# rust-cv/cv

Measured on NVIDIA H100. Metric: vSLAM frames/s (AKAZE+match+RANSAC, 1080p ~5k kp) at 1/2/4/8 H100, higher is better.
Workload: dtype f32+f64

## Files before the change

cv_b200/csrc/akaze.cu:

```cuda
#include <math.h>
#include <stdarg.h>
#include <stdio.h>
#include <stdlib.h>
#include <string.h>
#include <algorithm>
#include <vector>
#include "akaze_kernels.cuh"
#include "common.cuh"

using namespace akz;

namespace {

struct EvoHost {
    int w = 0, h = 0;
    uint32_t octave = 0, sublevel = 0;
    double esigma = 0, etime = 0;
    uint32_t sigma = 0;
    float quat = 0;
    float norm = 0, middle = 0;
    std::vector<double> tau;
    size_t off = 0;
    bool new_octave = false;
};
// ... 65 lines not shown
    int ks = radius * 2 + 1;
    if (ks > MAXK) return -1;
    t->ks = ks;
    memset(t->k, 0, sizeof(t->k));
    gaussian_kernel_host(r, ks, t->k);
    return 0;
}

}

struct AkazeWorkspace {
    cvb_akaze_cfg cfg{};
    uint32_t w = 0, h = 0, batch = 0;
    std::vector<EvoHost> evo;
    EvoTable table{};
    size_t plane_floats = 0;
    size_t p0 = 0;
    unsigned capc = 0, capk = 0;
    Taps g0{}, g1{};
    float *img = nullptr;
    float *Lt = nullptr, *Lsm = nullptr, *Lx = nullptr, *Ly = nullptr, *Lflow = nullptr, *Ldet = nullptr;
    float *tmpA = nullptr, *tmpB = nullptr, *tmpC = nullptr;
    bool fuse_blur_scharr = true;
    bool fuse_det = true;
    double *g2 = nullptr;
    unsigned long long *gmax = nullptr;
    unsigned *hist = nullptr, *npoints = nullptr;
    double *kc = nullptr;
    float *inv_k = nullptr;
    int *evo_octave = nullptr;
    unsigned *rowcount = nullptr, *rowoff = nullptr, *ncand = nullptr;
    Cand *cand = nullptr;
    cvb_keypoint *cache = nullptr, *refined = nullptr, *sorted = nullptr;
    unsigned *ncache = nullptr, *nsorted = nullptr, *nvalid = nullptr, *rank = nullptr;
    unsigned char *keep = nullptr, *valid = nullptr, *ok = nullptr, *desc_tmp = nullptr;
    unsigned *overflow = nullptr;
    CUtensorMap *tmaps = nullptr;
    bool use_tma = false;
    int tma_mask = 3;
    SupScratch sup{};
    bool suppress_seq = false;
    bool suppress_par_only = false;
    unsigned *sup_fallback = nullptr;
    unsigned char *tile_evo = nullptr;
    MaskLayout mask_layout{};
    unsigned *extrema_mask = nullptr;
    bool deriv_v3 = true;
    OrientTables *ot = nullptr;
    DescTables *dt = nullptr;
    cvb_keypoint *kp_out = nullptr;
    unsigned char *desc_out = nullptr;
    unsigned *n_out = nullptr;
    unsigned cap_out = 0;
    std::vector<void *> allocs;
    bool has_run = false;
    cudaStream_t aux = nullptr;
    cudaEvent_t ev_fork[8] = {}, ev_join = nullptr;
    struct GraphEntry { const void *img; void *kp, *desc, *n; unsigned B, cap; cudaGraphExec_t exec; };
    std::vector<GraphEntry> graphs;
    uint64_t launches_per_graph = 0;
    bool use_graph = true;
    bool use_aux = true;
};

void akaze_workspace_free(AkazeWorkspace *ws) {
    if (!ws) return;
    for (auto &g : ws->graphs) cudaGraphExecDestroy(g.exec);
// ... 208 lines not shown
    if (ws && same_cfg(ws->cfg, *cfg) && ws->w == w && ws->h == h && ws->batch >= batch && ws->cap_out >= cap_out) return 0;
    if (ws) { cvb_wait(ctx, ctx->stream); akaze_workspace_free(ws); ctx->akaze = nullptr; }
    if (cfg->descriptor_channels < 1 || cfg->descriptor_channels > 3) return cvb_set_error(ctx, CVB_EINVAL, "descriptor_channels must be 1..3");
    if (cfg->contrast_factor_num_bins < 1 || cfg->contrast_factor_num_bins > 8192) return cvb_set_error(ctx, CVB_EUNSUPPORTED, "contrast_factor_num_bins must be 1..8192");
    if (cfg->num_sublevels < 1) return cvb_set_error(ctx, CVB_EINVAL, "num_sublevels must be >= 1");
    if (!(cfg->base_scale_offset > 0.0)) return cvb_set_error(ctx, CVB_EINVAL, "sigma must be > 0.0");
    ws = new AkazeWorkspace();
    ws->cfg = *cfg; ws->w = w; ws->h = h; ws->batch = batch; ws->cap_out = cap_out;
    int rc = build_workspace(ctx, ws, cfg, batch, w, h, cap_out);
    if (rc) { cvb_wait(ctx, ctx->stream); akaze_workspace_free(ws); return rc; }
    ctx->akaze = ws;
    return 0;
}

int build_workspace(cvb_ctx *ctx, AkazeWorkspace *ws, const cvb_akaze_cfg *cfg, uint32_t batch, uint32_t w, uint32_t h, unsigned cap_out) {
    int rc = plan_evolutions(ctx, ws);
    if (rc) return rc;
    if (make_gauss_taps((float)cfg->base_scale_offset, &ws->g0)) return cvb_set_error(ctx, CVB_EUNSUPPORTED, "base_scale_offset too large");
    make_gauss_taps(1.0f, &ws->g1);
    ws->p0 = (size_t)w * h;
    ws->capc = (unsigned)std::min<size_t>(std::max<size_t>(ws->p0 / 8, 4096), 1u << 20);
    ws->capk = (unsigned)std::min<size_t>(std::max<size_t>(ws->p0 / 32, 4096), 1u << 17);
    const size_t B = batch, PF = ws->plane_floats, R = (size_t)std::max(ws->table.total_rows, 1);
#define DA(p, n) do { rc = dalloc(ctx, ws, &ws->p, (n)); if (rc) return rc; } while (0)
    DA(img, B * ws->p0);
    DA(Lt, B * PF); DA(Lsm, B * PF); DA(Lx, B * PF); DA(Ly, B * PF); DA(Lflow, B * PF); DA(Ldet, B * PF);
    DA(tmpA, B * ws->p0); DA(tmpB, B * ws->p0); DA(tmpC, B * ws->p0);
    DA(g2, B * ws->p0);
    DA(gmax, B); DA(hist, B * cfg->contrast_factor_num_bins); DA(npoints, B); DA(kc, B); DA(inv_k, B * MAX_EVO);
    DA(evo_octave, MAX_EVO);
    DA(rowcount, B * R); DA(rowoff, B * R); DA(ncand, B);
    DA(cand, B * ws->capc);
    DA(cache, B * ws->capk); DA(refined, B * ws->capk); DA(sorted, B * ws->capk);
    DA(ncache, B); DA(nsorted, B); DA(nvalid, B); DA(rank, B * ws->capk);
    DA(keep, B * ws->capk); DA(valid, B * ws->capk); DA(ok, B * ws->capk); DA(desc_tmp, B * ws->capk * 64);
    DA(overflow, 1);
    {
        unsigned nbmax = 1;
        for (size_t i = 0; i < ws->evo.size(); i++) {
            float ratio = (float)(1u << ws->evo[i].octave), off = 0.5f * (ratio - 1.0f), size = ws->table.e[i].size;
            float cell = fmaxf(16.0f, ceilf(2.0f * size + 2.0f * off + 2.0f));
            unsigned nbx = (unsigned)((float)w / cell) + 3, nby = (unsigned)((float)h / cell) + 3;
            nbmax = std::max(nbmax, nbx * nby);
        }
        ws->sup.nbmax = nbmax;
        DA(sup.state, B * ws->capc); DA(sup.alive, B * ws->capc); DA(sup.rdy, B * ws->capc);
        DA(sup.key, B * ws->capc); DA(sup.rank, B * ws->capc); DA(sup.next, B * ws->capc);
        DA(sup.binA, B * nbmax); DA(sup.binB, B * nbmax);
        const char *env = getenv("CVB_SUPPRESS_SEQ");
        ws->suppress_seq = env && env[0] == '1';
        env = getenv("CVB_SUPPRESS_GLOBAL");
        ws->suppress_par_only = env && env[0] == '1';
        DA(sup_fallback, B);
        env = getenv("CVB_NO_GRAPH");
        ws->use_graph = !(env && env[0] == '1');
        env = getenv("CVB_NO_AUX_STREAM");
        ws->use_aux = !(env && env[0] == '1');
        env = getenv("CVB_NO_FUSE_BLUR");
        ws->fuse_blur_scharr = !(env && env[0] == '1');
        env = getenv("CVB_NO_FUSE_DET");
        ws->fuse_det = !(env && env[0] == '1');
        cudaStreamCreateWithFlags(&ws->aux, cudaStreamNonBlocking);
        for (auto &e : ws->ev_fork) cudaEventCreateWithFlags(&e, cudaEventDisableTiming);
        cudaEventCreateWithFlags(&ws->ev_join, cudaEventDisableTiming);
        cudaFuncSetAttribute(k_suppress_smem, cudaFuncAttributeMaxDynamicSharedMemorySize, (int)SUP_SMEM);
    }
    DA(ot, 1); DA(dt, 1);
    DA(tmaps, 3 * MAX_EVO);
    DA(kp_out, B * (size_t)cap_out); DA(desc_out, B * (size_t)cap_out * 64); DA(n_out, B);
#undef DA
    {
        const char *env = getenv("CVB_TMA");
        ws->use_tma = env ? env[0] == '1' : (CVB_TMA_DEFAULT != 0);
        if (const char *m = getenv("CVB_TMA_MASK")) ws->tma_mask = atoi(m);
        std::vector<CUtensorMap> hm(3 * MAX_EVO);
        memset(hm.data(), 0, sizeof(CUtensorMap) * hm.size());
        for (size_t i = 0; i < ws->evo.size() && ws->use_tma; i++) {
            const EvoHost &e = ws->evo[i];
            const int S = std::min<int>((int)e.sigma, 5);
            if ((int)e.sigma > 5) { ws->use_tma = false; break; }
            const float *src1 = (i == 0 ? ws->Lt : ws->Lsm) + e.off;
            const bool ok = make_tmap(&hm[i], src1, e.w, e.h, batch, PF, pitch3(S), SH3 + 2 * S)
                         && make_tmap(&hm[MAX_EVO + i], ws->Lx + e.off, e.w, e.h, batch, PF, pitch3(S), SH3 + 2 * S)
                         && make_tmap(&hm[2 * MAX_EVO + i], ws->Ly + e.off, e.w, e.h, batch, PF, pitch3(S), SH3 + 2 * S);
            if (!ok) ws->use_tma = false;
        }
        CVB_CUDA(ctx, cudaMemcpyAsync(ws->tmaps, hm.data(), sizeof(CUtensorMap) * hm.size(), cudaMemcpyHostToDevice, ctx->stream));
        CVB_CUDA(ctx, cvb_wait(ctx, ctx->stream));
    }
    {
        std::vector<unsigned char> te((size_t)std::max(ws->table.total_tiles, 1), 0);
        ws->deriv_v3 = true;
        for (size_t i = 0; i < ws->evo.size(); i++) {
            const int t0 = ws->table.e[i].tilebase, t1 = i + 1 < ws->evo.size() ? ws->table.e[i + 1].tilebase : ws->table.total_tiles;
            for (int t = t0; t < t1; t++) te[(size_t)t] = (unsigned char)i;
            if (ws->evo[i].sigma > 5) ws->deriv_v3 = false;
        }
        rc = dalloc(ctx, ws, &ws->tile_evo, te.size());
// ... 223 lines not shown
            cur = dst; cur_bs = dst_bs;
        }
    }
    if ((rc = issue_detector_response(octave_first, E))) return rc;
    if (forked) {
        CVB_CUDA(ctx, cudaEventRecord(ws->ev_join, ws->aux));
        CVB_CUDA(ctx, cudaStreamWaitEvent(st, ws->ev_join, 0));
    }
    {
        if (!fused_det) { CVB_PROF(ctx, "k_extrema_mask", 4.0 * ws->plane_floats * B);
        k_extrema_mask<<<dim3((unsigned)ws->table.total_tiles, 1, B), NT, 0, st>>>(ws->Ldet, PF, ws->table, ws->tile_evo, ws->mask_layout, thr,
                                                                                    ws->extrema_mask, ws->rowcount);
        CVB_LAUNCH_CHECK(ctx); }
        { CVB_PROF(ctx, "k_scan_rows", 0);
        k_scan_rows<<<B, 1024, 0, st>>>(ws->rowcount, ws->rowoff, ws->ncand, R);
        CVB_LAUNCH_CHECK(ctx); }
        { CVB_PROF(ctx, "k_extrema_emit", 0);
        k_extrema_emit<<<dim3(cdiv((unsigned)R * 32u, NT), 1, B), NT, 0, st>>>(ws->Ldet, PF, ws->table, ws->mask_layout, ws->extrema_mask, ws->rowcount,
                                                                                 ws->rowoff, ws->cand, ws->capc, ws->overflow);
        CVB_LAUNCH_CHECK(ctx); }
    }
    { CVB_PROF(ctx, "k_suppress", 0);
    if (ws->suppress_seq)
        k_suppress_seq<<<B, 1024, 0, st>>>(ws->cand, ws->ncand, ws->capc, ws->table, ws->cache, ws->ncache, ws->capk, ws->overflow);
    else {
        k_suppress_smem<<<B, 1024, SUP_SMEM, st>>>(ws->cand, ws->ncand, ws->rowoff, ws->capc, ws->table, ws->sup, ws->cache,
                                                   ws->ncache, ws->capk, ws->overflow, ws->sup_fallback);
        CVB_LAUNCH_CHECK(ctx);
        k_suppress_par<<<B, 1024, 0, st>>>(ws->cand, ws->ncand, ws->rowoff, ws->capc, ws->table, ws->sup, ws->cache, ws->ncache,
                                           ws->capk, ws->overflow, ws->suppress_par_only ? nullptr : ws->sup_fallback);
    }
    CVB_LAUNCH_CHECK(ctx); }
    const unsigned kp_blocks = (unsigned)ctx->num_sms * 2;
    const unsigned ichunks = std::min<unsigned>(cdiv(ws->capk, NT), 64u);
    CVB_CUDA(ctx, cudaMemsetAsync(ws->keep, 1, (size_t)B * ws->capk, st));
    { CVB_PROF(ctx, "k_filter_upper", 0);
    k_filter_upper<<<dim3(ichunks, 16, B), NT, 0, st>>>(ws->cache, ws->ncache, ws->capk, ws->keep);
    CVB_LAUNCH_CHECK(ctx); }
    { CVB_PROF(ctx, "k_refine_orient", 0);
    k_refine_orient<<<dim3(kp_blocks, B), NT, 0, st>>>(ws->cache, ws->ncache, ws->capk, ws->keep, ws->table, ws->Ldet, ws->Lx, ws->Ly, PF,
                                                       ws->ot, ws->refined, ws->valid);
    CVB_LAUNCH_CHECK(ctx); }
    CVB_CUDA(ctx, cudaMemsetAsync(ws->rank, 0, sizeof(unsigned) * (size_t)B * ws->capk, st));
    CVB_CUDA(ctx, cudaMemsetAsync(ws->nvalid, 0, sizeof(unsigned) * B, st));
    { CVB_PROF(ctx, "k_rank_sort", 0);
    k_rank_count<<<dim3(ichunks, 16, B), NT, 0, st>>>(ws->refined, ws->valid, ws->ncache, ws->capk, ws->rank);
    CVB_LAUNCH_CHECK(ctx);
    k_rank_scatter<<<dim3(ichunks, B), NT, 0, st>>>(ws->refined, ws->valid, ws->ncache, ws->capk, ws->rank,
                                                    (long long)ws->cfg.maximum_features, ws->sorted, ws->nvalid);
    CVB_LAUNCH_CHECK(ctx);
    k_clamp_count<<<cdiv(B, 32), 32, 0, st>>>(ws->nvalid, (long long)ws->cfg.maximum_features, ws->nsorted, (int)B);
    CVB_LAUNCH_CHECK(ctx); }
    { CVB_PROF(ctx, "k_descriptors", 0);
    k_descriptors<<<dim3((unsigned)ctx->num_sms * 8, B), DESC_WARPS * 32, 0, st>>>(ws->sorted, ws->nsorted, ws->capk, ws->table, ws->Lt, ws->Lx,
                                                     ws->Ly, PF, ws->dt, (int)ws->cfg.descriptor_channels,
                                                     (int)ws->cfg.descriptor_pattern_size, ws->desc_tmp, ws->ok);
    CVB_LAUNCH_CHECK(ctx); }
    { CVB_PROF(ctx, "k_compact_final", 0);
    k_compact_final<<<B, 1024, 0, st>>>(ws->sorted, ws->desc_tmp, ws->ok, ws->nsorted, ws->capk, kp_out, desc_out, cap_out, n_out,
                                        ws->overflow);
    CVB_LAUNCH_CHECK(ctx); }
    ws->has_run = true;
    return 0;
}

int run_extract(cvb_ctx *ctx, const float *images, unsigned B, cvb_keypoint *kp_out, unsigned char *desc_out,
                unsigned cap_out, unsigned *n_out) {
    AkazeWorkspace *ws = ctx->akaze;
    if (!ws->use_graph || ctx->prof || ws->evo.empty()) return run_extract_eager(ctx, images, B, kp_out, desc_out, cap_out, n_out);
    for (auto &g : ws->graphs)
        if (g.img == images && g.kp == kp_out && g.desc == desc_out && g.n == n_out && g.B == B && g.cap == cap_out) {
            CVB_CUDA(ctx, cudaGraphLaunch(g.exec, ctx->stream));
            ctx->launches += ws->launches_per_graph;
            ws->has_run = true;
            return 0;
        }
    const uint64_t l0 = ctx->launches;
    cudaGraph_t graph = nullptr;
    CVB_CUDA(ctx, cudaStreamBeginCapture(ctx->stream, cudaStreamCaptureModeThreadLocal));
    int rc = run_extract_eager(ctx, images, B, kp_out, desc_out, cap_out, n_out);
    cudaError_t ce = cudaStreamEndCapture(ctx->stream, &graph);
    if (rc) { if (graph) cudaGraphDestroy(graph); return rc; }
    if (ce != cudaSuccess || !graph) {
        cudaGetLastError();
// ... 59 lines not shown
    CVB_CUDA(ctx, cudaMemcpyAsync(hs, ws->overflow, sizeof(unsigned), cudaMemcpyDeviceToHost, ctx->stream));
    CVB_CUDA(ctx, cudaMemsetAsync(ws->overflow, 0, sizeof(unsigned), ctx->stream));
    CVB_CUDA(ctx, cvb_wait(ctx, ctx->stream));
    *flag_out = hs[0];
    return 0;
}

int cvb_akaze_extract_batch(cvb_ctx *ctx, const cvb_akaze_cfg *cfg, const float *images, uint32_t batch, uint32_t w, uint32_t h,
                            cvb_keypoint *kp_out, uint8_t *desc_out, uint32_t cap, uint32_t *n_out) {
    return akaze_extract_batch_host(ctx, cfg, images, false, batch, w, h, kp_out, desc_out, cap, n_out);
}

}

int akaze_extract_batch_host(cvb_ctx *ctx, const cvb_akaze_cfg *cfg, const float *images, bool images_on_device, uint32_t batch, uint32_t w,
                             uint32_t h, cvb_keypoint *kp_out, uint8_t *desc_out, uint32_t cap, uint32_t *n_out) {
    int rc = check_args(ctx, cfg, images, batch, w, h);
    if (rc) return rc;
    if (!n_out || (cap && (!kp_out || !desc_out))) return cvb_set_error(ctx, CVB_EINVAL, "null output");
    CVB_CUDA(ctx, cudaSetDevice(ctx->device));
    rc = ensure_workspace(ctx, cfg, batch, w, h, std::max<uint32_t>(cap, 1));
    if (rc) return rc;
    AkazeWorkspace *ws = ctx->akaze;
    cudaStream_t st = ctx->stream;
    if (!images_on_device) CVB_CUDA(ctx, cudaMemcpyAsync(ws->img, images, sizeof(float) * ws->p0 * batch, cudaMemcpyHostToDevice, st));
    const unsigned cap_dev = ws->cap_out;
    rc = run_extract(ctx, images_on_device ? images : ws->img, batch, ws->kp_out, ws->desc_out, cap_dev, ws->n_out);
    if (rc) return rc;
    unsigned *hs = (unsigned *)cvb_pinned(ctx, sizeof(unsigned) * ((size_t)batch + 1));
    if (!hs) return cvb_set_error(ctx, CVB_ENOMEM, "page-locked scratch");
    CVB_CUDA(ctx, cudaMemcpyAsync(hs, ws->n_out, sizeof(unsigned) * batch, cudaMemcpyDeviceToHost, st));
    CVB_CUDA(ctx, cudaMemcpyAsync(hs + batch, ws->overflow, sizeof(unsigned), cudaMemcpyDeviceToHost, st));
    CVB_CUDA(ctx, cvb_wait(ctx, st));
    const unsigned ovf = hs[batch];
    for (uint32_t b = 0; b < batch; b++) n_out[b] = hs[b];
    if (ovf) {
        cudaMemsetAsync(ws->overflow, 0, sizeof(unsigned), st);
        if (ovf == 3) return cvb_set_error(ctx, CVB_ECAP, "output capacity %u too small", cap);
        return cvb_set_error(ctx, CVB_ECAP, "internal keypoint capacity exceeded (stage %u)", ovf);
    }
    for (uint32_t b = 0; b < batch; b++) {
        unsigned n = std::min<unsigned>(n_out[b], cap);
        if (!n) continue;
        CVB_CUDA(ctx, cudaMemcpyAsync(kp_out + (size_t)b * cap, ws->kp_out + (size_t)b * cap_dev, sizeof(cvb_keypoint) * n,
                                      cudaMemcpyDeviceToHost, st));
        CVB_CUDA(ctx, cudaMemcpyAsync(desc_out + (size_t)b * cap * 64, ws->desc_out + (size_t)b * cap_dev * 64, (size_t)n * 64,
                                      cudaMemcpyDeviceToHost, st));
    }
    CVB_CUDA(ctx, cvb_wait(ctx, st));
    return 0;
}

extern "C" {

int cvb_akaze_extract(cvb_ctx *ctx, const cvb_akaze_cfg *cfg, const float *image, uint32_t w, uint32_t h, cvb_keypoint *kp_out,
                      uint8_t *desc_out, uint32_t cap, uint32_t *n_out) {
    return cvb_akaze_extract_batch(ctx, cfg, image, 1, w, h, kp_out, desc_out, cap, n_out);
}

int cvb_akaze_debug_num_evolutions(cvb_ctx *ctx, uint32_t *n_out) {
    if (!ctx || !n_out) return CVB_EINVAL;
    if (!ctx->akaze || !ctx->akaze->has_run) return cvb_set_error(ctx, CVB_EINVAL, "no extract call yet");
    *n_out = (uint32_t)ctx->akaze->evo.size();
    return 0;
}

int cvb_akaze_debug_evolution(cvb_ctx *ctx, uint32_t i, uint32_t *w, uint32_t *h, uint32_t *octave, uint32_t *sigma_size,
                              uint32_t *n_fed_steps) {
// ... 45 lines not shown
        if (n) CVB_CUDA(ctx, cudaMemcpy(c.data(), ws->cand + (size_t)frame * ws->capc, sizeof(Cand) * n, cudaMemcpyDeviceToHost));
        for (unsigned i = 0; i < n; i++) {
            cvb_keypoint k{};
            const EvoHost &e = ws->evo[(size_t)c[i].e];
            k.x = (float)c[i].x; k.y = (float)c[i].y; k.response = fabsf(c[i].v);
            k.size = (float)(e.esigma * ws->cfg.derivative_factor); k.angle = 0.f; k.octave = e.octave; k.class_id = (uint32_t)c[i].e;
            res.push_back(k);
        }
    } else if (stage == 1 || stage == 2) {
        unsigned n = 0;
        CVB_CUDA(ctx, cudaMemcpy(&n, ws->ncache + frame, sizeof(unsigned), cudaMemcpyDeviceToHost));
        std::vector<cvb_keypoint> k(n);
        std::vector<unsigned char> f(n);
        const cvb_keypoint *src = stage == 1 ? ws->cache : ws->refined;
        const unsigned char *flg = stage == 1 ? ws->keep : ws->valid;
        if (n) {
            CVB_CUDA(ctx, cudaMemcpy(k.data(), src + (size_t)frame * ws->capk, sizeof(cvb_keypoint) * n, cudaMemcpyDeviceToHost));
            CVB_CUDA(ctx, cudaMemcpy(f.data(), flg + (size_t)frame * ws->capk, n, cudaMemcpyDeviceToHost));
        }
        for (unsigned i = 0; i < n; i++)
            if (f[i]) res.push_back(k[i]);
    } else if (stage == 3) {
        unsigned n = 0;
        CVB_CUDA(ctx, cudaMemcpy(&n, ws->nsorted + frame, sizeof(unsigned), cudaMemcpyDeviceToHost));
        res.resize(n);
        if (n) CVB_CUDA(ctx, cudaMemcpy(res.data(), ws->sorted + (size_t)frame * ws->capk, sizeof(cvb_keypoint) * n, cudaMemcpyDeviceToHost));
    } else return cvb_set_error(ctx, CVB_EINVAL, "bad stage");
    *n_out = (uint32_t)res.size();
    if (out)
        for (size_t i = 0; i < res.size() && i < cap; i++) out[i] = res[i];
    return 0;
}

}
```

cv_b200/csrc/akaze_kernels.cuh:

```cuda
#pragma once
#include <cuda.h>
#include <cuda/barrier>
#include <cuda_runtime.h>
#include <stdint.h>
#include "device_libm.cuh"
#include "../../include/cvb200.h"

namespace akz {

constexpr int TW = 32;
constexpr int TH = 32;
constexpr int NT = 256;
constexpr int MAXK = 33;
constexpr int MAX_EVO = 32;
constexpr int MAX_TAU = 64;
constexpr int FED_SMAX = 8, FED_FUSE_DEFAULT = 8;

struct Taps { int ks; float k[MAXK]; };

struct EvoDev {
    int w, h;
    unsigned long long off;
    int octave;
    float size;
// ... 1344 lines not shown
            const unsigned ex = block_excl_scan_1024(v, s_warp, &tot);
            if (g < ce) s_rank[g & M] = (unsigned short)(carry + ex);
            carry += tot;
        }
        __syncthreads();
        for (unsigned g = cs + threadIdx.x; g < ce; g += 1024) {
            const unsigned r = g & M;
            if (s_alive[r] && s_key[r] >= BASE) s_key[r] = N + (unsigned)s_rank[(cs + (s_key[r] - BASE)) & M];
        }
        N += carry;
        for (unsigned g = prev_cs + threadIdx.x; g < prev_ce; g += 1024) { g_alive[g] = s_alive[g & M]; g_key[g] = s_key[g & M]; }
        __syncthreads();
        prev_cs = cs; prev_ce = ce; prev_off = off; prev_ratio = ratio;
    }
    for (unsigned g = prev_cs + threadIdx.x; g < prev_ce; g += 1024) { g_alive[g] = s_alive[g & M]; g_key[g] = s_key[g & M]; }
    __syncthreads();
    for (unsigned g = threadIdx.x; g < ntot; g += 1024) {
        if (!g_alive[g]) continue;
        const unsigned k = g_key[g];
        if (k >= capk) { *overflow = 2u; continue; }
        const Cand c = cd[g];
        const EvoDev ev = T.e[c.e];
        const float ratio = (float)(1 << ev.octave);
        cvb_keypoint kp;
        kp.x = (float)c.x * ratio + 0.5f * (ratio - 1.0f);
        kp.y = (float)c.y * ratio + 0.5f * (ratio - 1.0f);
        kp.response = fabsf(c.v); kp.size = ev.size; kp.angle = 0.f;
        kp.octave = (uint32_t)ev.octave; kp.class_id = (uint32_t)c.e;
        cache[(size_t)b * capk + k] = kp;
    }
    if (threadIdx.x == 0) ncache[b] = min(N, capk);
}

__global__ void __launch_bounds__(NT) k_filter_upper(const cvb_keypoint *__restrict__ cache,
                                                     const unsigned *__restrict__ ncache, unsigned capk,
                                                     unsigned char *__restrict__ keep) {
    __shared__ float s_x[NT], s_y[NT], s_r[NT];
    __shared__ unsigned s_c[NT];
    __shared__ unsigned s_lo[NT / 32], s_hi[NT / 32];
    const int b = blockIdx.z;
    const unsigned n = ncache[b];
    const cvb_keypoint *kc = cache + (size_t)b * capk;
    const unsigned nchunks = (n + NT - 1) / NT;
    for (unsigned ic = blockIdx.x; ic < nchunks; ic += gridDim.x) {
        const unsigned i = ic * NT + threadIdx.x;
        cvb_keypoint a = {};
        if (i < n) a = kc[i];
        unsigned lo = i < n ? a.class_id : 0xffffffffu, hi = i < n ? a.class_id : 0u;
        lo = __reduce_min_sync(0xffffffffu, lo); hi = __reduce_max_sync(0xffffffffu, hi);
        __syncthreads();
        if ((threadIdx.x & 31) == 0) { s_lo[threadIdx.x >> 5] = lo; s_hi[threadIdx.x >> 5] = hi; }
        __syncthreads();
        for (int k = 0; k < NT / 32; k++) { lo = min(lo, s_lo[k]); hi = max(hi, s_hi[k]); }
        const float s2 = a.size * a.size;
        bool rep = false;
        for (unsigned jc = ic + blockIdx.y; jc < nchunks; jc += gridDim.y) {
            const unsigned j = jc * NT + threadIdx.x;
            cvb_keypoint q = {};
            bool relevant = false;
            if (j < n) { q = kc[j]; relevant = q.class_id >= lo + 1 && q.class_id <= hi + 1; }
            if (!__syncthreads_or(relevant)) continue;
            if (j < n) { s_x[threadIdx.x] = q.x; s_y[threadIdx.x] = q.y; s_r[threadIdx.x] = q.response; s_c[threadIdx.x] = q.class_id; }
            __syncthreads();
            if (i >= n) continue;
            const unsigned lim = min((unsigned)NT, n - jc * NT);
            for (unsigned u = 0; u < lim; u++) {
                if (jc * NT + u <= i || s_c[u] != a.class_id + 1) continue;
                float dx = a.x - s_x[u], dy = a.y - s_y[u];
                float dist = dx * dx + dy * dy;
                if (dist <= s2 && a.response <= s_r[u]) rep = true;
            }
        }
        if (rep) keep[(size_t)b * capk + i] = 0;
    }
}

struct OrientTables {
    int nwin;
    float ang1[64];
    float ang2[64];
    int nn;
    signed char di[109], dj[109];
    float gw[109];
};

__global__ void __launch_bounds__(NT) k_refine_orient(const cvb_keypoint *__restrict__ cache,
                                                      const unsigned *__restrict__ ncache, unsigned capk,
                                                      const unsigned char *__restrict__ keep, EvoTable T,
                                                      const float *__restrict__ Ldet, const float *__restrict__ Lx,
                                                      const float *__restrict__ Ly, size_t bstride,
                                                      const OrientTables *__restrict__ OT,
                                                      cvb_keypoint *__restrict__ refined,
                                                      unsigned char *__restrict__ valid) {
    __shared__ float2 s_r[NT / 32][112];
    __shared__ uint2 s_m[NT / 32][112];
    __shared__ float s_a1[64], s_a2[64];
    const int b = blockIdx.y;
    const unsigned n = ncache[b];
    const int lane = threadIdx.x & 31, wid = threadIdx.x >> 5;
    const float PI = 3.14159265358979323846f;
    const float two_pi = 2.0f * PI;
    const int nwin = OT->nwin, nn = OT->nn;
    if (threadIdx.x < 64) { s_a1[threadIdx.x] = OT->ang1[threadIdx.x]; s_a2[threadIdx.x] = OT->ang2[threadIdx.x]; }
    __syncthreads();
    auto count_lt = [](const float *A, int cnt, float v, int g) {
        g = min(max(g, 0), cnt);
// ... 70 lines not shown
            const int sh = wa & 31;
            float sxa = 0.f, sya = 0.f, sxb = 0.f, syb = 0.f;
#pragma unroll 4
            for (int k = 0; k < 109; k++) {
                const unsigned mb = mw[2 * k] >> sh;
                const float2 r = s_r[wid][k];
                if (mb & 1u) { sxa += r.x; sya += r.y; }
                if (mb & 2u) { sxb += r.x; syb += r.y; }
            }
            if (wa < nwin) {
                const float va = sxa * sxa + sya * sya;
                if (va > best_val) { best_val = va; best_sx = sxa; best_sy = sya; best_w = wa; }
            }
            if (wb < nwin) {
                const float vb = sxb * sxb + syb * syb;
                if (vb > best_val) { best_val = vb; best_sx = sxb; best_sy = syb; best_w = wb; }
            }
        }
        for (int o = 16; o; o >>= 1) {
            float ov = __shfl_xor_sync(0xffffffffu, best_val, o);
            float osx = __shfl_xor_sync(0xffffffffu, best_sx, o), osy = __shfl_xor_sync(0xffffffffu, best_sy, o);
            int ow = __shfl_xor_sync(0xffffffffu, best_w, o);
            if (ov > best_val || (ov == best_val && ow < best_w)) { best_val = ov; best_sx = osx; best_sy = osy; best_w = ow; }
        }
        if (lane == 0) {
            kp.angle = best_val > 0.f ? dlm::fast_atan2_equiv(best_sy, best_sx) : 0.f;
            refined[gi] = kp;
            valid[gi] = 1;
        }
        __syncwarp();
    }
}

__global__ void __launch_bounds__(NT) k_rank_count(const cvb_keypoint *__restrict__ refined,
                                                   const unsigned char *__restrict__ valid,
                                                   const unsigned *__restrict__ ncache, unsigned capk,
                                                   unsigned *__restrict__ rank) {
    __shared__ float s_r[NT];
    const int b = blockIdx.z;
    const unsigned n = ncache[b];
    const cvb_keypoint *kp = refined + (size_t)b * capk;
    const unsigned char *vl = valid + (size_t)b * capk;
    const unsigned nchunks = (n + NT - 1) / NT;
    for (unsigned ic = blockIdx.x; ic < nchunks; ic += gridDim.x)
        for (unsigned jc = blockIdx.y; jc < nchunks; jc += gridDim.y) {
            const unsigned i = ic * NT + threadIdx.x, j = jc * NT + threadIdx.x;
            __syncthreads();
            s_r[threadIdx.x] = (j < n && vl[j]) ? kp[j].response : -1.0f;
            __syncthreads();
            if (i >= n || !vl[i]) continue;
            const float ri = kp[i].response;
            const unsigned lim = min((unsigned)NT, n - jc * NT);
            unsigned cnt = 0;
            for (unsigned u = 0; u < lim; u++) {
                const float rj = s_r[u];
                if (rj > ri || (rj == ri && (jc * NT + u) < i)) cnt++;
            }
            if (cnt) atomicAdd(&rank[(size_t)b * capk + i], cnt);
        }
}

__global__ void __launch_bounds__(NT) k_rank_scatter(const cvb_keypoint *__restrict__ refined,
                                                     const unsigned char *__restrict__ valid,
                                                     const unsigned *__restrict__ ncache, unsigned capk,
                                                     const unsigned *__restrict__ rank, long long max_features,
                                                     cvb_keypoint *__restrict__ sorted, unsigned *__restrict__ nvalid) {
    const int b = blockIdx.y;
    const unsigned n = ncache[b];
    unsigned cnt = 0;
    for (unsigned i = blockIdx.x * NT + threadIdx.x; i < n; i += gridDim.x * NT) {
        if (!valid[(size_t)b * capk + i]) continue;
        cnt++;
        const unsigned r = rank[(size_t)b * capk + i];
        if (max_features < 0 || (long long)r < max_features) sorted[(size_t)b * capk + r] = refined[(size_t)b * capk + i];
    }
    for (int o = 16; o; o >>= 1) cnt += __shfl_down_sync(0xffffffffu, cnt, o);
    if ((threadIdx.x & 31) == 0 && cnt) atomicAdd(&nvalid[b], cnt);
}

__global__ void k_clamp_count(const unsigned *__restrict__ nvalid, long long max_features, unsigned *__restrict__ nsorted, int B) {
    const int b = blockIdx.x * blockDim.x + threadIdx.x;
    if (b >= B) return;
    unsigned v = nvalid[b];
    if (max_features >= 0 && (long long)v > max_features) v = (unsigned)max_features;
    nsorted[b] = v;
}

struct DescTables {
    int ncells;
    short ci[32], cj[32], cstep[32];
    int nbits;
    int nlat;
    unsigned char ba[512], bb[512], bch[512];
};

constexpr int DESC_WARPS = 4;
constexpr int DESC_MAXLAT = 21;

__global__ void __launch_bounds__(DESC_WARPS * 32) k_descriptors(const cvb_keypoint *__restrict__ sorted,
                                                    const unsigned *__restrict__ nsorted, unsigned capk, EvoTable T,
                                                    const float *__restrict__ Lt, const float *__restrict__ Lx,
                                                    const float *__restrict__ Ly, size_t bstride,
                                                    const DescTables *__restrict__ DT, int nch, int pattern,
                                                    unsigned char *__restrict__ desc_tmp,
                                                    unsigned char *__restrict__ ok) {
    __shared__ float s_val[DESC_WARPS][32][3];
    __shared__ float s_lat[DESC_WARPS][3][DESC_MAXLAT * DESC_MAXLAT];
    const int b = blockIdx.y;
    const unsigned n = nsorted[b];
    const int lane = threadIdx.x & 31, wid = threadIdx.x >> 5;
    const int nl = DT->nlat;
    for (unsigned q = blockIdx.x * DESC_WARPS + wid; q < n; q += gridDim.x * DESC_WARPS) {
        const size_t gi = (size_t)b * capk + q;
        const cvb_keypoint kp = sorted[gi];
        const EvoDev ev = T.e[kp.class_id];
        const size_t poff = (size_t)b * bstride + ev.off;
        const float *PT = Lt + poff, *PX = Lx + poff, *PY = Ly + poff;
        const int W = ev.w, H = ev.h;
// ... 131 lines not shown
```

Baseline: 1545.

## Replace quadratic keypoint filter and rank sort with bucketed filter and radix sort

The O(n^2) upper-level duplicate filter is replaced by a single-block kernel that buckets keypoints by class and y-band using counting sort, then checks only neighbouring bands. The O(n^2) pairwise rank-count sort plus its scatter and clamp kernels are replaced by a single-block-per-image 4-pass LSD radix sort held in shared memory, with a global-scratch fallback for large counts. This removes the quadratic work, several memsets and launches. In exchange, each image now runs on one 1024-thread block, which limits parallelism, and the band-based neighbour search assumes the cell size covers the suppression radius.

```diff
diff --git a/cv_b200/csrc/akaze.cu b/cv_b200/csrc/akaze.cu
--- a/cv_b200/csrc/akaze.cu
+++ b/cv_b200/csrc/akaze.cu
@@ -121,7 +121,8 @@
     unsigned *rowcount = nullptr, *rowoff = nullptr, *ncand = nullptr;
     Cand *cand = nullptr;
     cvb_keypoint *cache = nullptr, *refined = nullptr, *sorted = nullptr;
-    unsigned *ncache = nullptr, *nsorted = nullptr, *nvalid = nullptr, *rank = nullptr;
+    unsigned *ncache = nullptr, *nsorted = nullptr;
+    float4 *kp_scratch = nullptr;
     unsigned char *keep = nullptr, *valid = nullptr, *ok = nullptr, *desc_tmp = nullptr;
     unsigned *overflow = nullptr;
     CUtensorMap *tmaps = nullptr;
@@ -396,7 +397,7 @@
     DA(rowcount, B * R); DA(rowoff, B * R); DA(ncand, B);
     DA(cand, B * ws->capc);
     DA(cache, B * ws->capk); DA(refined, B * ws->capk); DA(sorted, B * ws->capk);
-    DA(ncache, B); DA(nsorted, B); DA(nvalid, B); DA(rank, B * ws->capk);
+    DA(ncache, B); DA(nsorted, B); DA(kp_scratch, B * ws->capk);
     DA(keep, B * ws->capk); DA(valid, B * ws->capk); DA(ok, B * ws->capk); DA(desc_tmp, B * ws->capk * 64);
     DA(overflow, 1);
     {
@@ -428,6 +429,7 @@
         for (auto &e : ws->ev_fork) cudaEventCreateWithFlags(&e, cudaEventDisableTiming);
         cudaEventCreateWithFlags(&ws->ev_join, cudaEventDisableTiming);
         cudaFuncSetAttribute(k_suppress_smem, cudaFuncAttributeMaxDynamicSharedMemorySize, (int)SUP_SMEM);
+        cudaFuncSetAttribute(k_sort_keypoints, cudaFuncAttributeMaxDynamicSharedMemorySize, (int)SORT_SMEM);
     }
     DA(ot, 1); DA(dt, 1);
     DA(tmaps, 3 * MAX_EVO);
@@ -717,24 +719,16 @@
     }
     CVB_LAUNCH_CHECK(ctx); }
     const unsigned kp_blocks = (unsigned)ctx->num_sms * 2;
-    const unsigned ichunks = std::min<unsigned>(cdiv(ws->capk, NT), 64u);
-    CVB_CUDA(ctx, cudaMemsetAsync(ws->keep, 1, (size_t)B * ws->capk, st));
     { CVB_PROF(ctx, "k_filter_upper", 0);
-    k_filter_upper<<<dim3(ichunks, 16, B), NT, 0, st>>>(ws->cache, ws->ncache, ws->capk, ws->keep);
+    k_filter_upper<<<B, 1024, 0, st>>>(ws->cache, ws->ncache, ws->capk, ws->table, ws->kp_scratch, ws->keep);
     CVB_LAUNCH_CHECK(ctx); }
     { CVB_PROF(ctx, "k_refine_orient", 0);
     k_refine_orient<<<dim3(kp_blocks, B), NT, 0, st>>>(ws->cache, ws->ncache, ws->capk, ws->keep, ws->table, ws->Ldet, ws->Lx, ws->Ly, PF,
                                                        ws->ot, ws->refined, ws->valid);
     CVB_LAUNCH_CHECK(ctx); }
-    CVB_CUDA(ctx, cudaMemsetAsync(ws->rank, 0, sizeof(unsigned) * (size_t)B * ws->capk, st));
-    CVB_CUDA(ctx, cudaMemsetAsync(ws->nvalid, 0, sizeof(unsigned) * B, st));
-    { CVB_PROF(ctx, "k_rank_sort", 0);
-    k_rank_count<<<dim3(ichunks, 16, B), NT, 0, st>>>(ws->refined, ws->valid, ws->ncache, ws->capk, ws->rank);
-    CVB_LAUNCH_CHECK(ctx);
-    k_rank_scatter<<<dim3(ichunks, B), NT, 0, st>>>(ws->refined, ws->valid, ws->ncache, ws->capk, ws->rank,
-                                                    (long long)ws->cfg.maximum_features, ws->sorted, ws->nvalid);
-    CVB_LAUNCH_CHECK(ctx);
-    k_clamp_count<<<cdiv(B, 32), 32, 0, st>>>(ws->nvalid, (long long)ws->cfg.maximum_features, ws->nsorted, (int)B);
+    { CVB_PROF(ctx, "k_sort_keypoints", 0);
+    k_sort_keypoints<<<B, 1024, SORT_SMEM, st>>>(ws->refined, ws->valid, ws->ncache, ws->capk, (long long)ws->cfg.maximum_features,
+                                                 reinterpret_cast<unsigned *>(ws->kp_scratch), ws->sorted, ws->nsorted);
     CVB_LAUNCH_CHECK(ctx); }
     { CVB_PROF(ctx, "k_descriptors", 0);
     k_descriptors<<<dim3((unsigned)ctx->num_sms * 8, B), DESC_WARPS * 32, 0, st>>>(ws->sorted, ws->nsorted, ws->capk, ws->table, ws->Lt, ws->Lx,
@@ -860,8 +854,11 @@
     CVB_CUDA(ctx, cudaMemcpyAsync(hs, ws->n_out, sizeof(unsigned) * batch, cudaMemcpyDeviceToHost, st));
     CVB_CUDA(ctx, cudaMemcpyAsync(hs + batch, ws->overflow, sizeof(unsigned), cudaMemcpyDeviceToHost, st));
     CVB_CUDA(ctx, cvb_wait(ctx, st));
-    const unsigned ovf = hs[batch];
-    for (uint32_t b = 0; b < batch; b++) n_out[b] = hs[b];
+    unsigned ovf = hs[batch];
+    for (uint32_t b = 0; b < batch; b++) {
+        n_out[b] = hs[b];
+        if (hs[b] > cap && !ovf) ovf = 3;
+    }
     if (ovf) {
         cudaMemsetAsync(ws->overflow, 0, sizeof(unsigned), st);
         if (ovf == 3) return cvb_set_error(ctx, CVB_ECAP, "output capacity %u too small", cap);
@@ -973,4 +970,28 @@
     return 0;
 }
 
-}
+int cvbk_sort_keypoints(cvb_ctx *ctx, const cvb_keypoint *refined_dev, const uint8_t *valid_dev, const uint32_t *ncache_dev,
+                        uint32_t batch, uint32_t capk, long long max_features, uint32_t *scratch_dev, cvb_keypoint *sorted_dev,
+                        uint32_t *nsorted_dev) {
+    if (!ctx || !batch) return CVB_EINVAL;
+    CVB_CUDA(ctx, cudaFuncSetAttribute(k_sort_keypoints, cudaFuncAttributeMaxDynamicSharedMemorySize, (int)SORT_SMEM));
+    k_sort_keypoints<<<batch, 1024, SORT_SMEM, ctx->stream>>>(refined_dev, valid_dev, ncache_dev, capk, max_features, scratch_dev,
+                                                              sorted_dev, nsorted_dev);
+    CVB_LAUNCH_CHECK(ctx);
+    CVB_CUDA(ctx, cvb_wait(ctx, ctx->stream));
+    return 0;
+}
+
+int cvbk_filter_upper(cvb_ctx *ctx, const cvb_keypoint *cache_dev, const uint32_t *ncache_dev, uint32_t batch, uint32_t capk,
+                      const float *class_size, uint32_t nclass, uint32_t height, float *scratch_dev, uint8_t *keep_dev) {
+    if (!ctx || !batch || !class_size || nclass < 1 || nclass > (uint32_t)MAX_EVO || !height) return CVB_EINVAL;
+    EvoTable T{};
+    T.n = (int)nclass;
+    for (uint32_t c = 0; c < nclass; c++) { T.e[c].size = class_size[c]; T.e[c].h = (int)height; }
+    k_filter_upper<<<batch, 1024, 0, ctx->stream>>>(cache_dev, ncache_dev, capk, T, reinterpret_cast<float4 *>(scratch_dev), keep_dev);
+    CVB_LAUNCH_CHECK(ctx);
+    CVB_CUDA(ctx, cvb_wait(ctx, ctx->stream));
+    return 0;
+}
+
+}
diff --git a/cv_b200/csrc/akaze_kernels.cuh b/cv_b200/csrc/akaze_kernels.cuh
--- a/cv_b200/csrc/akaze_kernels.cuh
+++ b/cv_b200/csrc/akaze_kernels.cuh
@@ -1400,46 +1400,72 @@
     if (threadIdx.x == 0) ncache[b] = min(N, capk);
 }
 
-__global__ void __launch_bounds__(NT) k_filter_upper(const cvb_keypoint *__restrict__ cache,
-                                                     const unsigned *__restrict__ ncache, unsigned capk,
-                                                     unsigned char *__restrict__ keep) {
-    __shared__ float s_x[NT], s_y[NT], s_r[NT];
-    __shared__ unsigned s_c[NT];
-    __shared__ unsigned s_lo[NT / 32], s_hi[NT / 32];
-    const int b = blockIdx.z;
-    const unsigned n = ncache[b];
+constexpr int FU_ROWS = 256;
+__global__ void __launch_bounds__(1024) k_filter_upper(const cvb_keypoint *__restrict__ cache,
+                                                       const unsigned *__restrict__ ncache, unsigned capk, EvoTable T,
+                                                       float4 *__restrict__ bucketed, unsigned char *__restrict__ keep) {
+    __shared__ unsigned s_off[MAX_EVO * FU_ROWS];
+    __shared__ float s_cell[MAX_EVO];
+    __shared__ unsigned s_nrow[MAX_EVO];
+    __shared__ unsigned s_warp[33];
+    const int b = blockIdx.x;
+    const unsigned n = ncache[b], E = (unsigned)T.n, NB = E * FU_ROWS;
     const cvb_keypoint *kc = cache + (size_t)b * capk;
-    const unsigned nchunks = (n + NT - 1) / NT;
-    for (unsigned ic = blockIdx.x; ic < nchunks; ic += gridDim.x) {
-        const unsigned i = ic * NT + threadIdx.x;
-        cvb_keypoint a = {};
-        if (i < n) a = kc[i];
-        unsigned lo = i < n ? a.class_id : 0xffffffffu, hi = i < n ? a.class_id : 0u;
-        lo = __reduce_min_sync(0xffffffffu, lo); hi = __reduce_max_sync(0xffffffffu, hi);
-        __syncthreads();
-        if ((threadIdx.x & 31) == 0) { s_lo[threadIdx.x >> 5] = lo; s_hi[threadIdx.x >> 5] = hi; }
-        __syncthreads();
-        for (int k = 0; k < NT / 32; k++) { lo = min(lo, s_lo[k]); hi = max(hi, s_hi[k]); }
-        const float s2 = a.size * a.size;
+    float4 *bk = bucketed + (size_t)b * capk;
+    const float hmax = (float)T.e[0].h;
+    if (threadIdx.x >= 1 && threadIdx.x < E) {
+        const float cell = fmaxf(T.e[threadIdx.x - 1].size + 1.0f, hmax / (float)(FU_ROWS - 2));
+        s_cell[threadIdx.x] = cell;
+        s_nrow[threadIdx.x] = min((unsigned)(hmax / cell) + 2u, (unsigned)FU_ROWS);
+    }
+    for (unsigned k = threadIdx.x; k < NB; k += 1024) s_off[k] = 0;
+    __syncthreads();
+    auto band = [&](unsigned c, float y) -> unsigned {
+        const float q = floorf(y / s_cell[c]);
+        const unsigned r = q > 0.f ? (unsigned)fminf(q, (float)(FU_ROWS - 1)) : 0u;
+        return c * FU_ROWS + min(r, s_nrow[c] - 1);
+    };
+    for (unsigned j = threadIdx.x; j < n; j += 1024) {
+        const unsigned c = kc[j].class_id;
+        if (c >= 1 && c < E) atomicAdd(&s_off[band(c, kc[j].y)], 1u);
+    }
+    __syncthreads();
+    unsigned carry = 0;
+    for (unsigned base = 0; base < NB; base += 1024) {
+        const unsigned k = base + threadIdx.x;
+        const unsigned v = k < NB ? s_off[k] : 0u;
+        unsigned tot;
+        const unsigned ex = block_excl_scan_1024(v, s_warp, &tot);
+        if (k < NB) s_off[k] = carry + ex;
+        carry += tot;
+    }
+    __syncthreads();
+    for (unsigned j = threadIdx.x; j < n; j += 1024) {
+        const cvb_keypoint q = kc[j];
+        if (q.class_id >= 1 && q.class_id < E) {
+            const unsigned p = atomicAdd(&s_off[band(q.class_id, q.y)], 1u);
+            bk[p] = make_float4(q.x, q.y, q.response, __uint_as_float(j));
+        }
+    }
+    __syncthreads();
+    for (unsigned i = threadIdx.x; i < n; i += 1024) {
+        const cvb_keypoint a = kc[i];
+        const unsigned c = a.class_id + 1;
         bool rep = false;
-        for (unsigned jc = ic + blockIdx.y; jc < nchunks; jc += gridDim.y) {
-            const unsigned j = jc * NT + threadIdx.x;
-            cvb_keypoint q = {};
-            bool relevant = false;
-            if (j < n) { q = kc[j]; relevant = q.class_id >= lo + 1 && q.class_id <= hi + 1; }
-            if (!__syncthreads_or(relevant)) continue;
-            if (j < n) { s_x[threadIdx.x] = q.x; s_y[threadIdx.x] = q.y; s_r[threadIdx.x] = q.response; s_c[threadIdx.x] = q.class_id; }
-            __syncthreads();
-            if (i >= n) continue;
-            const unsigned lim = min((unsigned)NT, n - jc * NT);
-            for (unsigned u = 0; u < lim; u++) {
-                if (jc * NT + u <= i || s_c[u] != a.class_id + 1) continue;
-                float dx = a.x - s_x[u], dy = a.y - s_y[u];
+        if (c < E) {
+            const unsigned k = band(c, a.y), r = k - c * FU_ROWS;
+            const unsigned lo = r > 0 ? k - 1 : k, hi = r + 1 < s_nrow[c] ? k + 1 : k;
+            const unsigned end = s_off[hi];
+            const float s2 = a.size * a.size;
+            for (unsigned p = lo > 0 ? s_off[lo - 1] : 0u; p < end; p++) {
+                const float4 q = bk[p];
+                if (__float_as_uint(q.w) <= i) continue;
+                float dx = a.x - q.x, dy = a.y - q.y;
                 float dist = dx * dx + dy * dy;
-                if (dist <= s2 && a.response <= s_r[u]) rep = true;
-            }
-        }
-        if (rep) keep[(size_t)b * capk + i] = 0;
+                if (dist <= s2 && a.response <= q.z) { rep = true; break; }
+            }
+        }
+        keep[(size_t)b * capk + i] = rep ? 0 : 1;
     }
 }
 
@@ -1576,58 +1602,92 @@
     }
 }
 
-__global__ void __launch_bounds__(NT) k_rank_count(const cvb_keypoint *__restrict__ refined,
-                                                   const unsigned char *__restrict__ valid,
-                                                   const unsigned *__restrict__ ncache, unsigned capk,
-                                                   unsigned *__restrict__ rank) {
-    __shared__ float s_r[NT];
-    const int b = blockIdx.z;
+constexpr unsigned SORT_SMEM_CAP = 14336;
+constexpr int SORT_WC_PITCH = 33;
+constexpr size_t SORT_SMEM = (4 * 256 + 256 * SORT_WC_PITCH + 64) * sizeof(unsigned) +
+                             (size_t)SORT_SMEM_CAP * 2 * (sizeof(unsigned) + sizeof(unsigned short));
+
+template <typename I>
+__device__ void sort_desc_body(const cvb_keypoint *__restrict__ kp, const unsigned char *__restrict__ vl, unsigned n,
+                               long long max_features, cvb_keypoint *__restrict__ out, unsigned *__restrict__ nout,
+                               unsigned *s_hist, unsigned *s_wc, unsigned *s_warp, unsigned *k0, I *i0, unsigned *k1, I *i1) {
+    const unsigned t = threadIdx.x, lane = t & 31, wid = t >> 5;
+    s_hist[t] = 0;
+    __syncthreads();
+    unsigned m = 0;
+    for (unsigned base = 0; base < n; base += 1024) {
+        const unsigned i = base + t;
+        const unsigned v = i < n && vl[i] ? 1u : 0u;
+        unsigned tot;
+        const unsigned ex = block_excl_scan_1024(v, s_warp, &tot);
+        if (v) {
+            const unsigned key = ~__float_as_uint(kp[i].response);
+            k0[m + ex] = key; i0[m + ex] = (I)i;
+            for (int p = 0; p < 4; p++) atomicAdd(&s_hist[p * 256 + ((key >> (8 * p)) & 255u)], 1u);
+        }
+        m += tot;
+    }
+    __syncthreads();
+    {
+        const unsigned v = s_hist[t];
+        unsigned x = v;
+        for (int o = 1; o < 32; o <<= 1) { const unsigned y = __shfl_up_sync(0xffffffffu, x, o); if (lane >= o) x += y; }
+        if (lane == 31) s_warp[wid] = x;
+        __syncthreads();
+        unsigned off = 0;
+        for (unsigned w = wid & ~7u; w < wid; w++) off += s_warp[w];
+        s_hist[t] = off + x - v;
+        __syncthreads();
+    }
+    for (int p = 0; p < 4; p++) {
+        const int sh = 8 * p;
+        for (unsigned base = 0; base < m; base += 1024) {
+            const unsigned e = base + t;
+            const bool has = e < m;
+            const unsigned key = has ? k0[e] : 0u;
+            const unsigned d = (key >> sh) & 255u;
+            for (unsigned k = t; k < 256 * SORT_WC_PITCH; k += 1024) s_wc[k] = 0;
+            __syncthreads();
+            const unsigned peers = __match_any_sync(0xffffffffu, has ? d : 0x100u);
+            const unsigned rank = __popc(peers & ((1u << lane) - 1u));
+            if (has && rank == 0) s_wc[d * SORT_WC_PITCH + wid] = __popc(peers);
+            __syncthreads();
+            if (t < 256) {
+                unsigned run = s_hist[p * 256 + t];
+                for (int w = 0; w < 32; w++) { const unsigned c = s_wc[t * SORT_WC_PITCH + w]; s_wc[t * SORT_WC_PITCH + w] = run; run += c; }
+                s_hist[p * 256 + t] = run;
+            }
+            __syncthreads();
+            if (has) { const unsigned q = s_wc[d * SORT_WC_PITCH + wid] + rank; k1[q] = key; i1[q] = i0[e]; }
+            __syncthreads();
+        }
+        unsigned *tk = k0; k0 = k1; k1 = tk;
+        I *ti = i0; i0 = i1; i1 = ti;
+    }
+    const unsigned cnt = (max_features >= 0 && (long long)m > max_features) ? (unsigned)max_features : m;
+    for (unsigned r = t; r < cnt; r += 1024) out[r] = kp[i0[r]];
+    if (t == 0) *nout = cnt;
+}
+
+__global__ void __launch_bounds__(1024) k_sort_keypoints(const cvb_keypoint *__restrict__ refined,
+                                                         const unsigned char *__restrict__ valid,
+                                                         const unsigned *__restrict__ ncache, unsigned capk, long long max_features,
+                                                         unsigned *__restrict__ scratch, cvb_keypoint *__restrict__ sorted,
+                                                         unsigned *__restrict__ nsorted) {
+    extern __shared__ __align__(16) unsigned sort_sm[];
+    const int b = blockIdx.x;
     const unsigned n = ncache[b];
-    const cvb_keypoint *kp = refined + (size_t)b * capk;
-    const unsigned char *vl = valid + (size_t)b * capk;
-    const unsigned nchunks = (n + NT - 1) / NT;
-    for (unsigned ic = blockIdx.x; ic < nchunks; ic += gridDim.x)
-        for (unsigned jc = blockIdx.y; jc < nchunks; jc += gridDim.y) {
-            const unsigned i = ic * NT + threadIdx.x, j = jc * NT + threadIdx.x;
-            __syncthreads();
-            s_r[threadIdx.x] = (j < n && vl[j]) ? kp[j].response : -1.0f;
-            __syncthreads();
-            if (i >= n || !vl[i]) continue;
-            const float ri = kp[i].response;
-            const unsigned lim = min((unsigned)NT, n - jc * NT);
-            unsigned cnt = 0;
-            for (unsigned u = 0; u < lim; u++) {
-                const float rj = s_r[u];
-                if (rj > ri || (rj == ri && (jc * NT + u) < i)) cnt++;
-            }
-            if (cnt) atomicAdd(&rank[(size_t)b * capk + i], cnt);
-        }
-}
-
-__global__ void __launch_bounds__(NT) k_rank_scatter(const cvb_keypoint *__restrict__ refined,
-                                                     const unsigned char *__restrict__ valid,
-                                                     const unsigned *__restrict__ ncache, unsigned capk,
-                                                     const unsigned *__restrict__ rank, long long max_features,
-                                                     cvb_keypoint *__restrict__ sorted, unsigned *__restrict__ nvalid) {
-    const int b = blockIdx.y;
-    const unsigned n = ncache[b];
-    unsigned cnt = 0;
-    for (unsigned i = blockIdx.x * NT + threadIdx.x; i < n; i += gridDim.x * NT) {
-        if (!valid[(size_t)b * capk + i]) continue;
-        cnt++;
-        const unsigned r = rank[(size_t)b * capk + i];
-        if (max_features < 0 || (long long)r < max_features) sorted[(size_t)b * capk + r] = refined[(size_t)b * capk + i];
-    }
-    for (int o = 16; o; o >>= 1) cnt += __shfl_down_sync(0xffffffffu, cnt, o);
-    if ((threadIdx.x & 31) == 0 && cnt) atomicAdd(&nvalid[b], cnt);
-}
-
-__global__ void k_clamp_count(const unsigned *__restrict__ nvalid, long long max_features, unsigned *__restrict__ nsorted, int B) {
-    const int b = blockIdx.x * blockDim.x + threadIdx.x;
-    if (b >= B) return;
-    unsigned v = nvalid[b];
-    if (max_features >= 0 && (long long)v > max_features) v = (unsigned)max_features;
-    nsorted[b] = v;
+    unsigned *s_hist = sort_sm, *s_wc = s_hist + 4 * 256, *s_warp = s_wc + 256 * SORT_WC_PITCH, *s_data = s_warp + 64;
+    const size_t o = (size_t)b * capk;
+    if (n <= SORT_SMEM_CAP) {
+        unsigned short *si = reinterpret_cast<unsigned short *>(s_data + 2 * SORT_SMEM_CAP);
+        sort_desc_body<unsigned short>(refined + o, valid + o, n, max_features, sorted + o, nsorted + b, s_hist, s_wc, s_warp,
+                                       s_data, si, s_data + SORT_SMEM_CAP, si + SORT_SMEM_CAP);
+    } else {
+        unsigned *g = scratch + 4 * o;
+        sort_desc_body<unsigned>(refined + o, valid + o, n, max_features, sorted + o, nsorted + b, s_hist, s_wc, s_warp,
+                                 g, g + capk, g + 2 * (size_t)capk, g + 3 * (size_t)capk);
+    }
 }
 
 struct DescTables {
```

New measurement: 1557 (median of 6 runs). Within noise of the previous version (+0.8%).
